# DCDmllm/AnyEdit

Hardware: AMD Instinct MI355X
Metric: edited-images/sec @512x512, 50 DDIM steps (higher is better)
Workload: dtype bf16; 1 GPU; configs[1]: AnySD (SD-1.5 UNet in=8 + task embedding/expert adapters) 512x512 bf16, 50 DDIM steps, batch=4/GPU, 3-branch CFG (UNet batch 12); images_per_gpu=4, ddim_steps=50, cfg_branches=3, hip_graph=True, parallelism=dp1 (image-sharded, no data-path collective)

## Files before the change

anyedit_amd/_lib.py:

```python
import ctypes
import os

import torch

_HERE = os.path.dirname(os.path.abspath(__file__))
LIB_PATH = os.environ.get("AE_LIB_PATH") or os.path.join(_HERE, "libanyedit_hip.so")

c_void_p, c_int, c_long, c_float = ctypes.c_void_p, ctypes.c_int, ctypes.c_long, ctypes.c_float

SIGNATURES = {
    "ae_version": [],
    "ae_last_error": [],
    "ae_device_arch": [ctypes.c_char_p, c_int],
    "ae_device_info": [ctypes.POINTER(c_int), ctypes.POINTER(c_long), ctypes.POINTER(c_int)],
    "ae_gemm_bf16": [c_void_p, c_long, c_void_p, c_long, c_int, c_void_p, c_long, c_void_p, c_long, c_int, c_int, c_int,
                     c_void_p, c_void_p, c_long, c_void_p, c_long, c_int, c_int, c_int, c_void_p, c_void_p],
    "ae_conv3x3_workspace_floats": [c_int, c_int, c_int, c_int, c_int, c_int, c_int],
    "ae_conv3x3_partials_bf16": [c_void_p, c_void_p, c_int, c_int, c_int, c_int, c_int, c_void_p, c_int, c_void_p, c_void_p],
    "ae_groupnorm_splitk_supported": [c_int, c_int, c_int, c_int, c_int],
    "ae_groupnorm_splitk_nhwc_bf16": [c_void_p, c_int, c_void_p, c_void_p, c_long, c_void_p, c_void_p, c_void_p, c_int, c_int, c_int, c_int, c_float, c_int, c_void_p],
    "ae_conv3x3_bf16": [c_void_p, c_void_p, c_void_p, c_void_p, c_long, c_void_p, c_void_p, c_int, c_int, c_int, c_int, c_int,
                        c_int, c_int, c_int, c_void_p, c_void_p, c_int, c_void_p],
    "ae_conv3x3_up2_bf16": [c_void_p, c_void_p, c_void_p, c_void_p, c_int, c_int, c_int, c_int, c_int, c_void_p, c_void_p],
    "ae_groupnorm_rows_per_chunk": [c_int, c_int],
# ... 16 lines not shown
    "ae_add_bf16": [c_void_p, c_void_p, c_void_p, c_long, c_void_p],
    "ae_axpy_bf16": [c_void_p, c_void_p, c_float, c_void_p, c_long, c_void_p],
    "ae_geglu_fwd_bf16": [c_void_p, c_void_p, c_long, c_int, c_void_p],
    "ae_geglu_bwd_bf16": [c_void_p, c_void_p, c_void_p, c_long, c_int, c_void_p],
    "ae_sumpool2x2_bf16": [c_void_p, c_void_p, c_int, c_int, c_int, c_int, c_void_p],
    "ae_colsum_bf16_f32": [c_void_p, c_void_p, c_int, c_int, c_long, c_void_p],
    "ae_mse_grad_f32": [c_void_p, c_void_p, c_void_p, c_long, c_float, c_void_p],
    "ae_adamw_f32": [c_void_p, c_void_p, c_void_p, c_void_p, c_long, c_float, c_float, c_float, c_float, c_float, c_int, c_float,
                     c_void_p],
    "ae_rowsum_f32": [c_void_p, c_void_p, c_int, c_long, c_void_p],
    "ae_scatter_add_rows_f32": [c_void_p, c_void_p, c_void_p, c_int, c_int, c_int, c_void_p],
    "ae_attn_fp8_workspace_bytes": [c_int, c_int, c_int, c_int, c_int],
    "ae_attn_fwd_fp8": [c_void_p, c_void_p, c_void_p, c_void_p, c_int, c_int, c_int, c_int, c_int] + [c_long] * 12 +
                       [c_float, c_void_p, c_void_p, c_int, c_int, c_void_p, c_long, c_void_p],
    "ae_ln_gemm_supported": [c_int, c_int, c_int, c_int],
    "ae_ln_gemm_bf16": [c_void_p, c_long, c_void_p, c_long, c_void_p, c_long, c_int, c_int, c_int, c_void_p, c_void_p, c_long, c_void_p, c_void_p,
                        c_float, c_int, c_void_p, c_void_p],
    "ae_gemm_ln_plan": [c_int, c_int, c_int, c_int, c_int],
    "ae_xattn_fused_supported": [c_int, c_int, c_int, c_int, c_int, c_int, c_int],
    "ae_xattn_fused_covers": [c_int, c_int, c_int, c_int, c_int, c_int, c_int],
    "ae_xattn_fused_kv_bytes": [],
    "ae_xattn_fused_bf16": [c_void_p, c_long, c_void_p, c_void_p, c_float, c_void_p, c_void_p, c_void_p, c_void_p, c_void_p, c_void_p, c_long, c_int, c_int, c_int, c_int,
                            c_float, c_void_p],
    "ae_ff_fused_supported": [c_int, c_int, c_int],
    "ae_ff_fused_bf16": [c_void_p, c_long, c_void_p, c_void_p, c_float, c_void_p, c_long, c_void_p, c_void_p, c_void_p, c_void_p, c_long,
                         c_void_p, c_long, c_void_p, c_void_p, c_long, c_void_p, c_void_p, c_long, c_int, c_int, c_int, c_void_p],
    "ae_gemm_ln_bf16": [c_void_p, c_long, c_void_p, c_long, c_void_p, c_long, c_int, c_int, c_int, c_void_p, c_void_p, c_long, c_int, c_void_p,
                        c_void_p, c_int, c_void_p, c_float, c_void_p],
    "ae_task_gate_bwd": [c_void_p, c_void_p, c_void_p, c_void_p, c_int, c_int, c_int, c_void_p, c_void_p],
    "ae_task_gate_wgrad": [c_void_p, c_void_p, c_void_p, c_void_p, c_void_p, c_int, c_int, c_int, c_int, c_void_p, c_void_p, c_void_p],
    "ae_expert_kv_fwd": [c_void_p, c_void_p, c_void_p, c_void_p, c_int, c_int, c_int, c_int, c_int, c_void_p],
    "ae_expert_kv_dgrad_slices": [c_int],
    "ae_expert_kv_dgrad": [c_void_p, c_void_p, c_void_p, c_void_p, c_int, c_int, c_int, c_int, c_int, c_void_p, c_void_p],
    "ae_expert_kv_wgrad": [c_void_p, c_void_p, c_void_p, c_void_p, c_int, c_int, c_int, c_int, c_int, c_void_p],
    "ae_transpose_last2": [c_void_p, c_void_p, c_int, c_int, c_int, c_int, c_int, c_int, c_void_p],
    "ae_concat_channels_bf16": [c_void_p, c_int, c_void_p, c_int, c_void_p, c_long, c_void_p],
    "ae_im2col3x3_c8_bf16": [c_void_p, c_void_p, c_int, c_int, c_int, c_void_p],
    "ae_split_channels_bf16": [c_void_p, c_int, c_int, c_void_p, c_void_p, c_long, c_int, c_int, c_void_p],
    "ae_timestep_embedding": [c_void_p, c_void_p, c_void_p, c_void_p, c_int, c_int, c_float, c_void_p],
    "ae_ddim_step_f32": [c_void_p, c_void_p, c_void_p, c_void_p, c_void_p, c_void_p, c_long, c_int, c_float, c_float, c_float,
                         c_float, c_float, c_float, c_float, c_float, c_void_p],
    "ae_ddim_encode_step_f32": [c_void_p, c_void_p, c_void_p, c_long, c_int, c_float, c_float, c_float, c_void_p],
    "ae_plms_combine_f32": [c_void_p, c_void_p, c_void_p, c_void_p, c_void_p, c_long, c_int, c_void_p],
    "ae_mask_blend_f32": [c_void_p, c_void_p, c_void_p, c_void_p, c_void_p, c_int, c_int, c_int, c_float, c_float, c_int, c_void_p],
    "ae_q_sample_f32": [c_void_p, c_void_p, c_void_p, c_void_p, c_void_p, c_int, c_long, c_void_p],
    "ae_silu_to_bf16": [c_void_p, c_int, c_void_p, c_long, c_void_p],
# ... 12 lines not shown
    "ae_ms_deform_attn_bwd_f32": [c_void_p] * 9 + [c_int] * 7 + [c_void_p],
    "ae_linear_f32": [c_void_p, c_long, c_void_p, c_long, c_void_p, c_void_p, c_long, c_int, c_int, c_int, c_void_p],
    "ae_dpm_multistep_f32": [c_void_p] * 5 + [c_long, c_int, c_float, c_int, c_int, c_float, c_float, c_int, c_float, c_float, c_float,
                             c_float, c_void_p],
    "ae_layernorm_act_bf16": [c_void_p, c_void_p, c_void_p, c_void_p, c_long, c_int, c_float, c_int, c_void_p],
    "ae_sam_pe_encode_f32": [c_void_p, c_void_p, c_void_p, c_void_p, c_void_p, c_int, c_int, c_float, c_float, c_float, c_void_p],
    "ae_sam_mask_downscale_bf16": [c_void_p] * 10 + [c_int, c_int, c_int, c_float, c_void_p],
    "ae_sam_mask_product_f32": [c_void_p, c_void_p, c_void_p, c_int, c_int, c_int, c_int, c_int, c_void_p],
    "ae_sam_postprocess_masks": [c_void_p, c_void_p, c_void_p] + [c_int] * 8 + [c_float, c_int, c_void_p],
    "ae_nms_sorted_f32": [c_void_p, c_void_p, c_int, c_float, c_void_p],
    "ae_sam_preprocess_f32": [c_void_p, c_int, c_void_p, c_int, c_int, c_int, c_int, c_int, c_void_p, c_void_p, c_void_p],
    "ae_patchify_f32_bf16": [c_void_p, c_void_p, c_int, c_int, c_int, c_int, c_int, c_void_p],
    "ae_mse_f32": [c_void_p, c_void_p, c_void_p, c_long, c_void_p],
    "ae_lincomb4_f32": [c_void_p, c_void_p, c_float, c_void_p, c_float, c_void_p, c_float, c_void_p, c_float, c_long, c_void_p],
    "ae_dpm_adaptive_err_f32": [c_void_p, c_void_p, c_void_p, c_float, c_float, c_int, c_long, c_void_p, c_void_p],
    "ae_task_gate": [c_void_p, c_void_p, c_void_p, c_void_p, c_int, c_int, c_int, c_int, c_void_p, c_void_p, c_void_p, c_void_p],
    "ae_attn_causal_short_bf16": [c_void_p, c_void_p, c_void_p, c_void_p, c_int, c_int, c_int, c_int] + [c_long] * 12 + [c_float, c_void_p],
    "ae_clip_embed_bf16": [c_void_p, c_int, c_void_p, c_void_p, c_void_p, c_int, c_int, c_int, c_int, c_int, c_void_p],
    "ae_bias_act_f32_bf16": [c_void_p, c_long, c_void_p, c_void_p, c_long, c_long, c_int, c_int, c_void_p],
    "ae_clip_pool_eos_bf16": [c_void_p, c_int, c_void_p, c_void_p, c_int, c_int, c_int, c_long, c_void_p],
}
_RESTYPES = {"ae_last_error": ctypes.c_char_p, "ae_groupnorm_workspace_floats": c_long, "ae_conv3x3_workspace_floats": c_long,
             "ae_groupnorm_bwd_workspace_floats": c_long, "ae_attn_fp8_workspace_bytes": c_long, "ae_attn_bwd_workspace_floats": c_long,
             "ae_xattn_fused_kv_bytes": c_long}


class AnyEditHipError(RuntimeError):
    pass


def _load():
    if not os.path.exists(LIB_PATH):
        raise ImportError(
            f"{LIB_PATH} is missing: the HIP extension is REQUIRED (no CPU/eager fallback exists). "
            "Build it with `python -c 'import __graft_entry__ as g; g.build()'` or `python anyedit_amd/build.py`.")
    lib = ctypes.CDLL(LIB_PATH)
    for name, argtypes in SIGNATURES.items():
        fn = getattr(lib, name)
        fn.argtypes = argtypes
        fn.restype = _RESTYPES.get(name, c_int)
    return lib


lib = _load()


def check(rc, what=""):
# ... 10 lines not shown
```

anyedit_amd/anysd/model.py:

```python
import torch
import torch.nn as nn

from anyedit_amd import ops
from anyedit_amd.cldm.model import trusted_torch_load
from anyedit_amd.ldm.modules.attention import BasicTransformerBlock

BF16 = torch.bfloat16

EDIT_TYPES = ["add", "remove", "replace", "color_alter", "appearance_alter", "material_alter", "action_change",
              "textual_change", "background_change", "tone_transfer", "style_change", "movement", "outpaint", "rotation_change",
              "resize", "implicit_change", "relation_change", "counting", "visual_reference", "visual_bbox", "visual_depth",
              "visual_scribble", "visual_segment", "visual_sketch", "visual_material_transfer"]


class ImageProjModel(nn.Module):

    def __init__(self, clip_dim=1280, cross_dim=768, tokens=4):
        super().__init__()
        self.tokens, self.cross_dim = tokens, cross_dim
        self.proj = nn.Linear(clip_dim, tokens * cross_dim)
        self.norm = nn.LayerNorm(cross_dim)

    def rows(self, ref_embeds):
        B = ref_embeds.shape[0]
# ... 34 lines not shown
    @torch.no_grad()
    def prepare_conditioning(self, encoder_hidden_states, ref_embeds, edit_code, ip_scale=None):
        B, L, Dc = encoder_hidden_states.shape
        dev = encoder_hidden_states.device
        te = self.task_embs.detach()[edit_code.long()]
        ctx = torch.cat([encoder_hidden_states.float(), te[:, None, :].float()], dim=1)
        context_rows = ctx.reshape(B * (L + 1), Dc).to(BF16).contiguous()
        probs, top1, top1p = self.route(edit_code)
        gate = top1p if ip_scale is None else top1p * ip_scale
        ip_rows = self.image_proj_model.rows(ref_embeds)
        T_ip = self.image_proj_model.tokens
        kv_cache = {}
        for blk, W in zip(self._blocks, self.adapter_modules):
            attn = blk.attn2
            kv_cache[id(attn)] = attn.project_kv(context_rows)
            Wm = W.detach()
            if Wm.dtype != torch.float32 or not Wm.is_contiguous():
                Wm = Wm.float().contiguous()
            kv_ip = ops.expert_kv(ip_rows, Wm, top1, T_ip)
            kv_cache[("adapter", id(attn))] = (kv_ip, gate.float().contiguous())
            img = attn.fused_kv_images(kv_cache[id(attn)], kv_cache[("adapter", id(attn))], B)
            if img is not None:
                kv_cache[("xattn_img", id(attn))] = img
        return context_rows, kv_cache

    @torch.no_grad()
    def denoise(self, x, timesteps, context_rows, kv_cache, emb_pack=None):
        return self.unet.forward_rows(x, timesteps, context_rows, kv_cache=kv_cache, emb_pack=emb_pack)

    def forward(self, noisy_latents, timesteps, encoder_hidden_states, image_embeds, edit_code):
        context_rows, kv_cache = self.prepare_conditioning(encoder_hidden_states, image_embeds, edit_code)
        return self.denoise(noisy_latents, timesteps, context_rows, kv_cache)
```

anyedit_amd/build.py:

```python
import hashlib
import os
import shutil
import subprocess
import sys

HERE = os.path.dirname(os.path.abspath(__file__))
CSRC = os.path.join(HERE, "csrc")
LIB = os.path.join(HERE, "libanyedit_hip.so")
SOURCES = ["c_api.hip", "gemm_conv.hip", "gemm_rowpanel.hip", "ff_fused.hip", "xattn_fused.hip", "attention.hip", "attention_fast.hip", "attention_fp8.hip", "attention_bwd.hip", "norm.hip", "elementwise.hip", "backward.hip", "gate.hip", "expert_kv.hip", "msda.hip",
           "sam_decoder.hip", "clip_text.hip"]
EXTRA = {"gemm_conv.hip": ["-fno-slp-vectorize"], "gemm_rowpanel.hip": ["-fno-slp-vectorize"], "ff_fused.hip": ["-fno-slp-vectorize"], "xattn_fused.hip": ["-fno-slp-vectorize"], "attention.hip": ["-ffinite-math-only"],
         "attention_fast.hip": ["-ffinite-math-only", "-fno-slp-vectorize"], "attention_fp8.hip": ["-ffinite-math-only"],
         "attention_bwd.hip": ["-ffinite-math-only"], "clip_text.hip": ["-ffinite-math-only"]}
FLAGS = ["--offload-arch=gfx950", "-O3", "-std=c++17", "-fPIC", "-fno-gpu-rdc", "-Wno-unused-result"]


def _hipcc():
    for c in (shutil.which("hipcc"), "/opt/rocm/bin/hipcc"):
        if c and os.path.exists(c):
            return c
    raise RuntimeError("hipcc not found: the HIP extension cannot be built")


def _digest():
    h = hashlib.sha256()
    for name in sorted(os.listdir(CSRC)):
        with open(os.path.join(CSRC, name), "rb") as f:
            h.update(name.encode() + f.read())
    h.update((" ".join(FLAGS) + repr(sorted(EXTRA.items()))).encode())
    return h.hexdigest()


def build_library(force=False, verbose=True, variant=None, extra_flags=None):
    lib = LIB if variant is None else os.path.join(HERE, f"libanyedit_hip_{variant}.so")
    extra = {k: list(v) for k, v in EXTRA.items()}
    for k, v in (extra_flags or {}).items():
# ... 46 lines not shown
```

anyedit_amd/ldm/modules/attention.py:

```python
import os

import torch
import torch.nn as nn

from anyedit_amd import ops
from anyedit_amd.ldm.util import default, exists
from anyedit_amd.ldm.modules.diffusionmodules.util import Linear, Conv2d, LayerNorm, checkpoint

BF16 = torch.bfloat16
_XATTN_FUSED = os.environ.get("AE_XATTN_FUSED", "0") != "0"
_FF_TAIL = os.environ.get("AE_FF_TAIL", "1") != "0"
_SEG2_160 = os.environ.get("AE_ATTN_SEG2_160", "1") != "0"


def zero_module(module):
    for p in module.parameters():
        p.detach().zero_()
    return module


class _GN6(nn.GroupNorm):

    def _affine(self):
        if ops.cache_stale(self, "_pk", self.weight, self.bias):
            self._pk = (self.weight.detach().float().contiguous(), self.bias.detach().float().contiguous())
        return self._pk

    def repack(self):
        self._pk = None

    def rows(self, x, B, HW, colstats=None):
        g, b = self._affine()
        return ops.groupnorm(x, g, b, B, HW, self.eps, silu=False, groups=self.num_groups, colstats=colstats)
# ... 120 lines not shown
        if ops.cache_stale(self, "_pk", self.to_q.weight, self.to_k.weight, self.to_v.weight):
            wq, wk, wv = (ops.pack_linear(m.weight) for m in (self.to_q, self.to_k, self.to_v))
            pk = {"dev": self.to_q.weight.device, "q": wq, "kv": torch.cat([wk, wv], 0).contiguous()}
            if wq.shape[1] == wk.shape[1]:
                pk["qkv"] = torch.cat([wq, wk, wv], 0).contiguous()
            self._pk = pk
        return self._pk

    def _packed_x(self):
        if ops.cache_stale(self, "_pkx", self.to_q.weight, self.to_out[0].weight, self.to_out[0].bias):
            bo = self.to_out[0].bias
            self._pkx = (ops.pack_xattn_wq(self.to_q.weight), ops.pack_xattn_wo(self.to_out[0].weight), None if bo is None else bo.detach().float().contiguous())
        return self._pkx

    def fused_kv_images(self, kv, adapter, B):
        if not _XATTN_FUSED or self.is_self or self.heads != 8 or self.dim_head != 40 or self.to_q.weight.shape[1] != 320:
            return None
        Nk = kv.shape[0] // B
        T = 0 if adapter is None else adapter[0].shape[0] // B
        if not (64 < Nk <= 80 and T <= 16):
            return None
        return ops.pack_xattn_kv(kv, None if adapter is None else adapter[0], B, Nk, T)

    def project_kv(self, ctx_rows):
        return ops.gemm(ctx_rows, self._packed()["kv"])

    def rows(self, x, B, N, context_rows=None, Nk=None, kv=None, key_mask=None, residual=None, adapter=None, norm=None, rowstats=None,
             out_rowstats=None, kv_img=None):
        h, d = self.heads, self.dim_head
        inner = h * d
        if kv_img is not None and kv is not None and norm is not None and residual is x and key_mask is None and out_rowstats is None:
            Nk_ = kv.shape[0] // B
            T_ = 0 if adapter is None else adapter[0].shape[0] // B
            if ops.xattn_fused_ok(x.shape[0], x.shape[1], h, d, N, Nk_, T_):
                wq_img, wo_img, bo = self._packed_x()
                g_, be_ = norm._affine()
                return ops.xattn_fused(x, g_, be_, norm.eps, wq_img, kv_img, None if adapter is None else adapter[1], wo_img, bo, N, Nk_, T_, self.scale)
        pk = self._packed()

        def proj(wname):
            if norm is None:
                return ops.gemm(x, pk[wname])
            if rowstats is not None and ops.ln_fold_plan(x.shape[0], pk[wname].shape[0], x.shape[1], ops.EPI_NONE, 2):
                wq, s, c = self._packed_ln(wname, norm)
                return ops.gemm_ln(x, rowstats, wq, s, c, norm.eps)
            g, be = norm._affine()
            return ops.ln_gemm(x, g, be, norm.eps, pk[wname])

        if context_rows is None and kv is None:
            qkv = proj("qkv")
            s = (N * 3 * inner, d, 3 * inner)
            o = ops.attention(qkv, qkv[:, inner:], qkv[:, 2 * inner:], B, h, N, N, d, self.scale, s, s, s, key_mask=key_mask)
        else:
            q = proj("q")
            if kv is None:
                kv = self.project_kv(context_rows)
            Nk = kv.shape[0] // B
            qs = (N * inner, d, inner)
            ks = (Nk * 2 * inner, d, 2 * inner)
            if adapter is not None and (d <= 96 or (d == 160 and _SEG2_160)) and key_mask is None:
                kv_ip, gate = adapter
                T_ip = kv_ip.shape[0] // B
                ks_ip = (T_ip * 2 * inner, d, 2 * inner)
                seg2 = (kv_ip, kv_ip[:, inner:], T_ip, ks_ip, ks_ip, gate)
                o = ops.attention(q, kv, kv[:, inner:], B, h, N, Nk, d, self.scale, qs, ks, ks, seg2=seg2)
            else:
                o = ops.attention(q, kv, kv[:, inner:], B, h, N, Nk, d, self.scale, qs, ks, ks, key_mask=key_mask)
                if adapter is not None:
                    kv_ip, gate = adapter
                    T_ip = kv_ip.shape[0] // B
                    ks_ip = (T_ip * 2 * inner, d, 2 * inner)
                    ops.attention(q, kv_ip, kv_ip[:, inner:], B, h, N, T_ip, d, self.scale, qs, ks_ip, ks_ip, out=o,
                                  out_scale=gate, accumulate=True)
        return self.to_out[0].rows(o.reshape(B * N, inner), residual=residual, rowstats=out_rowstats)

    def forward(self, x, context=None, mask=None):
        B, N, C = x.shape
        xr = x.reshape(B * N, C).to(BF16).contiguous()
        ctx = None
        if context is not None:
            ctx = context.reshape(-1, context.shape[-1]).to(BF16).contiguous()
        km = None
        if exists(mask):
# ... 59 lines not shown
        M, C = x.shape
        f1, f2, f3 = self._fold_plan(M, C)
        kv2, adapter, kv_img = None, None, None
        if kv_cache is not None and context_rows is not None and not (ops._TAPE is not None and ops._TAPE.active):
            kv_img = kv_cache.get(("xattn_img", id(self.attn2)))
        use_x = kv_img is not None and not f3 and ops.xattn_fused_ok(M, C, self.attn2.heads, self.attn2.dim_head, N, 78, 0)
        st2 = ops.rowstats_buffer(M, C, x.device) if (f2 and not use_x) else None
        st3 = ops.rowstats_buffer(M, C, x.device) if f3 else None
        x = self.attn1.rows(x, B, N, context_rows=c1, residual=x, norm=self.norm1, rowstats=rowstats if f1 else None, out_rowstats=st2)
        if kv_cache is not None and context_rows is not None:
            key = id(self.attn2)
            kv2 = kv_cache.get(key)
            if kv2 is None:
                kv2 = self.attn2.project_kv(context_rows)
                if not (ops._TAPE is not None and ops._TAPE.active):
                    kv_cache[key] = kv2
            adapter = kv_cache.get(("adapter", key))
            if callable(adapter):
                adapter = adapter()
            if kv_img is None and not f3 and not (ops._TAPE is not None and ops._TAPE.active):
                img = self.attn2.fused_kv_images(kv2, adapter, B)
                if img is not None:
                    kv_cache[("xattn_img", key)] = img
        x = self.attn2.rows(x, B, N, context_rows=context_rows, kv=kv2, residual=x, adapter=adapter, norm=self.norm2, rowstats=st2, out_rowstats=st3,
                            kv_img=kv_img if use_x else None)
        x = self.ff.rows(x, residual=x, norm=self.norm3, rowstats=st3, tail=tail)
        return x

    def forward(self, x, context=None):
        B, N, C = x.shape
        ctx = None if context is None else context.reshape(-1, context.shape[-1]).to(BF16).contiguous()
        y = self.rows(x.reshape(B * N, C).to(BF16).contiguous(), B, N, context_rows=ctx)
        return y.reshape(B, N, C).to(x.dtype)

    _forward = forward


class SpatialTransformer(nn.Module):

    def __init__(self, in_channels, n_heads, d_head, depth=1, dropout=0., context_dim=None, disable_self_attn=False,
                 use_linear=False, use_checkpoint=True):
        super().__init__()
        if exists(context_dim) and not isinstance(context_dim, list):
            context_dim = [context_dim] * depth
        if context_dim is None:
            context_dim = [None] * depth
        self.in_channels = in_channels
        inner_dim = n_heads * d_head
# ... 46 lines not shown
```

anyedit_amd/ops.py:

```python
import torch

import ctypes
import os
import threading

from ._lib import lib, check as _check

BF16 = torch.bfloat16
EPI_NONE, EPI_GELU, EPI_GEGLU, EPI_SILU, EPI_RELU = 0, 1, 2, 3, 4


def _s():
    return torch.cuda.current_stream().cuda_stream


def _p(t):
    return None if t is None else t.data_ptr()


_live = threading.local()


def _tmp(t):
    if t is not None:
# ... 281 lines not shown
    _chk(wo_img, BF16, "xattn_fused.wo_img", 3)
    _chk(kv_img, BF16, "xattn_fused.kv_img", 3)
    _chk(gamma, torch.float32, "xattn_fused.gamma", 1)
    _chk(beta, torch.float32, "xattn_fused.beta", 1)
    M, C = x.shape
    B = M // rows_per_sample
    if tuple(wq_img.shape) != (8, 48, 320) or tuple(wo_img.shape) != (4, 320, 112) or tuple(kv_img.shape) != (B, 8, 14848) or not (wq_img.is_contiguous() and wo_img.is_contiguous()
                                                                                                                                    and kv_img.is_contiguous()) or x.stride(1) != 1:
        raise ValueError(f"xattn_fused: x {tuple(x.shape)}, images {tuple(wq_img.shape)} / {tuple(wo_img.shape)} / {tuple(kv_img.shape)} do not fit together")
    if gate is not None:
        _chk(gate, torch.float32, "xattn_fused.gate", 1)
        if gate.numel() != B:
            raise ValueError("xattn_fused: one gate per sample")
    if bo is not None:
        _chk(bo, torch.float32, "xattn_fused.bo", 1)
    if out is None:
        out = torch.empty(M, C, dtype=BF16, device=x.device)
    _chk(out, BF16, "xattn_fused.out", 2)
    check(lib.ae_xattn_fused_bf16(_p(x), x.stride(0), _p(gamma), _p(beta), float(eps), _p(wq_img), _p(kv_img), _p(gate), _p(wo_img), _p(bo), _p(out), out.stride(0), M,
                                  rows_per_sample, Nk, T, float(scale), _s()), "ae_xattn_fused_bf16")
    return out


def colstats_buffer(M, N, device):
    return torch.empty((M + 31) // 32, N, 2, dtype=torch.float32, device=device)


_GN_COLSTATS = os.environ.get("AE_GN_COLSTATS", "1") != "0"


def want_colstats(HW):
    return _GN_COLSTATS and HW > 256 and HW % 32 == 0 and not (_TAPE is not None and _TAPE.active)


def gemm(a, w, bias=None, residual=None, addvec=None, rows_per_batch=0, epilogue=EPI_NONE, out_f32=False, a2=None, out=None, colstats=None,
         rowstats=None):
    if rowstats is not None:
        if _TAPE is not None and _TAPE.active:
            raise ValueError("gemm: row statistics are not recorded on the training tape (ln_fold_plan is False while it records)")
        if addvec is not None or a2 is not None or out_f32 or colstats is not None or epilogue != EPI_NONE:
            raise ValueError("gemm: rowstats goes with a plain bf16 GEMM (+bias, +residual) only")
        return _gemm_ln(a, w, bias, residual, EPI_NONE, out, rowstats, None, None, 0.0)
    if _TAPE is not None and _TAPE.active:
        return _TAPE.gemm(a, w, bias=bias, residual=residual, addvec=addvec, rows_per_batch=rows_per_batch, epilogue=epilogue, out_f32=out_f32, a2=a2, out=out)
    _chk(a, BF16, "gemm.a", 2)
    _chk(w, BF16, "gemm.w", 2)
# ... 1216 lines not shown
    return f"gemm_rowpanel_kernel<K=320,LN{',geglu' if epilogue == EPI_GEGLU else ''}>|M={M} N={N}", 2.0 * M * N * K, nb


def _gemm_ln_label(_r, a, w, bias, residual, epilogue, out, M, N, K, rowstats_out, ln_stats, nparts, ln_colsum, eps):
    nb = 2 * (M * K + N * K) + _r.numel() * 2 + (2 * M * N if residual is not None else 0)
    tag = "rowstats" if rowstats_out is not None else "LNfold"
    if _ROWPANEL and os.environ.get("AE_RP_FOLD", "1") != "0" and lib.ae_ln_gemm_supported(M, N, K, epilogue) and (rowstats_out is None or epilogue == EPI_NONE):
        return f"gemm_rowpanel_kernel<K=320,{tag}{',geglu' if epilogue == EPI_GEGLU else ''}>|M={M} N={N}", 2.0 * M * N * K, nb
    return f"gemm_kernel<{_tile_label(M, N, False, K, epilogue == EPI_GEGLU, True, xe2=rowstats_out is None)},dense,{tag}>|M={M} N={N} K={K}", 2.0 * M * N * K, float(nb)


def _up2_label(_r, x, w4, bias, B, H, W, **_):
    y = _r[0]
    M, Cout, Cin = x.shape[0], w4.shape[1], x.shape[1]
    t192 = (M // 192) * (Cout // 320) * 4 if (M % 192 == 0 and Cout % 320 == 0) else 0
    tl = "192x320" if t192 and t192 / (-(-t192 // 256) * 256) >= 0.85 else "128x128"
    nb = 2 * (x.numel() + 16 * Cin * Cout) + 2 * y.numel()
    return f"gemm_kernel<{tl},conv3x3,up2x2>|M={y.shape[0]} Cin={Cin} Cout={Cout}", 2.0 * y.shape[0] * Cout * 4 * Cin, float(nb)


conv3x3_up2 = _wrap_profiled(conv3x3_up2, _up2_label)
xattn_fused = _wrap_profiled(xattn_fused, lambda _r, x, gamma, beta, eps, wq_img, kv_img, gate, wo_img, bo, rows_per_sample, Nk, T, scale, out=None: (
    f"xattn_fused_kernel<C=320>|M={x.shape[0]} Nk={Nk}+{T}", 2.0 * x.shape[0] * 320 * (2 * 320 + 2 * (Nk + T)), float(2 * (3 * x.numel() + wq_img.numel() + wo_img.numel() + kv_img.numel()))))
ff_fused = _wrap_profiled(ff_fused, lambda _r, x, gamma, beta, eps, w1, b1, w2img, b2, residual=None, out=None, w3=None, b3=None, residual3=None, colstats=None: (
    f"ff_fused_kernel<C=320{',proj_out' if w3 is not None else ''}>|M={x.shape[0]} H={w1.shape[0] // 2}",
    2.0 * x.shape[0] * x.shape[1] * (3 * (w1.shape[0] // 2) + (x.shape[1] if w3 is not None else 0)),
    float(2 * (x.numel() * (2 + (residual is not None and residual is not x) + (residual3 is not None)) + w1.numel() + w2img.numel() + (w3.numel() if w3 is not None else 0))),
    2 if colstats is not None else 1))
_ln_gemm_fused = _wrap_profiled(_ln_gemm_launch, _ln_gemm_label)
_gemm_ln_launch = _wrap_profiled(_gemm_ln_launch, _gemm_ln_label)
gemm = _wrap_profiled(gemm, _gemm_label)
attention_fp8 = _wrap_profiled(attention_fp8, _attn8_label)
conv3x3 = _wrap_profiled(conv3x3, _conv_label)
conv3x3_partials = _wrap_profiled(conv3x3_partials, lambda _r, x, w, B, H, W, k_order=0: (
    f"gemm_kernel<{_tile_label(x.shape[0], w.shape[0], True, 9 * (-(-x.shape[1] // 64) * 64), False, x.shape[1] % 64 == 0)},conv3x3>|M={x.shape[0]} Cin={x.shape[1]} Cout={w.shape[0]} s1 partials",
    2.0 * x.shape[0] * w.shape[0] * 9 * x.shape[1], float(2 * (x.numel() + 9 * x.shape[1] * w.shape[0]) + 2 * x.shape[0] * w.shape[0]), 1))
groupnorm_splitk = _wrap_profiled(groupnorm_splitk, lambda _r, partials, *a, **k: (
    f"groupnorm(splitK fold)|rows={_r.shape[0]} C={_r.shape[1]}", 0.0, 2.0 * _r.numel() * 2, 1))
attention = _wrap_profiled(attention, _attn_label)
groupnorm = _wrap_profiled(groupnorm, _gn_label)
layernorm = _wrap_profiled(layernorm, _ln_label)
expert_kv = _wrap_profiled(expert_kv, lambda _r, x, W, experts, tokens: (
    f"expert_kv_fwd_kernel|rows={x.shape[0]} N={W.shape[1]} Dc={W.shape[2]}", 2.0 * x.shape[0] * W.shape[1] * W.shape[2], 4.0 * (x.shape[0] // tokens) * W.shape[1] * W.shape[2]))
expert_kv_dgrad = _wrap_profiled(expert_kv_dgrad, lambda _r, dy, W, experts, tokens: (
    f"expert_kv_dgrad_kernel|rows={dy.shape[0]} N={W.shape[1]} Dc={W.shape[2]}", 2.0 * dy.shape[0] * W.shape[1] * W.shape[2], 4.0 * (dy.shape[0] // tokens) * W.shape[1] * W.shape[2]))
expert_kv_wgrad = _wrap_profiled(expert_kv_wgrad, lambda _r, dy, x, experts, tokens, n_experts, out=None: (
# ... 2 lines not shown
```

include/anyedit_hip.h:

```cpp
#ifndef ANYEDIT_HIP_H
#define ANYEDIT_HIP_H

#ifdef __cplusplus
extern "C" {
#endif

#define AE_OK 0
#define AE_ERR_ARG (-1)
#define AE_ERR_LAUNCH (-2)
#define AE_ERR_UNSUPPORTED (-3)

#define AE_EPI_NONE 0
#define AE_EPI_GELU 1
#define AE_EPI_GEGLU 2
#define AE_EPI_SILU 3
#define AE_EPI_RELU 4

int ae_version(void);
const char* ae_last_error(void);
int ae_device_arch(char* buf, int n);
int ae_device_info(int* cus, long* hbm_bytes, int* clock_khz);

int ae_gemm_bf16(const void* A, long lda, const void* A2, long lda2, int Ksplit, const void* W, long ldw, void* C, long ldc,
                 int M, int N, int K, const float* bias, const void* residual, long ldr, const float* addvec, long addvec_ld,
                 int rows_per_batch, int epilogue, int out_f32, float* colstats, void* stream);

int ae_ln_gemm_supported(int M, int N, int K, int epilogue);
int ae_ln_gemm_bf16(const void* A, long lda, const void* W, long ldw, void* C, long ldc, int M, int N, int K, const float* bias,
                    const void* residual, long ldr, const float* ln_gamma, const float* ln_beta, float ln_eps, int epilogue,
                    float* colstats , void* stream);

int ae_gemm_ln_plan(int M, int N, int K, int epilogue, int mode);
int ae_gemm_ln_bf16(const void* A, long lda, const void* W, long ldw, void* C, long ldc, int M, int N, int K, const float* bias,
                    const void* residual, long ldr, int epilogue, float* rowstats_out, const float* ln_stats, int ln_parts,
                    const float* ln_colsum, float ln_eps, void* stream);

int ae_ff_fused_supported(int M, int C, int H);
int ae_ff_fused_bf16(const void* X, long ldx, const float* ln_gamma, const float* ln_beta, float ln_eps, const void* W1, long ldw1, const float* b1,
                     const void* W2img, const float* b2, const void* residual, long ldr, const void* W3, long ldw3, const float* b3,
                     const void* residual3, long ldr3, float* colstats, void* Y, long ldy, int M, int C, int H, void* stream);

int ae_xattn_fused_supported(int M, int C, int heads, int head_dim, int rows_per_sample, int Nk, int T);
int ae_xattn_fused_covers(int M, int C, int heads, int head_dim, int rows_per_sample, int Nk, int T);
long ae_xattn_fused_kv_bytes(void);
int ae_xattn_fused_bf16(const void* X, long ldx, const float* ln_gamma, const float* ln_beta, float ln_eps, const void* Wq_img, const void* KV_img, const float* gate,
                        const void* Wo_img, const float* bo, void* Y, long ldy, int M, int rows_per_sample, int Nk, int T, float scale, void* stream);

long ae_conv3x3_workspace_floats(int B, int H, int W, int Cin, int Cout, int stride, int upsample2x);
int ae_conv3x3_partials_bf16(const void* x, const void* w, int B, int H, int W, int Cin, int Cout, float* workspace, int k_order, int* splitk_out, void* stream);
int ae_conv3x3_bf16(const void* x, const void* w, const float* bias, const float* addvec, long addvec_ld, const void* residual,
                    void* y, int B, int H, int W, int Cin, int Cout, int stride, int upsample2x, int out_f32, float* workspace,
                    float* colstats , int k_order, void* stream);

int ae_conv3x3_up2_bf16(const void* x, const void* w4, const float* bias, void* y, int B, int H, int W, int Cin, int Cout,
                        float* colstats, void* stream);

int ae_groupnorm_rows_per_chunk(int HW, int C);
long ae_groupnorm_workspace_floats(int B, int HW, int C, int groups);
int ae_groupnorm_splitk_supported(int B, int HW, int C, int groups, int splitk);
int ae_groupnorm_splitk_nhwc_bf16(const float* partial, int splitk, const float* bias, const float* addvec, long addvec_ld, const float* gamma, const float* beta,
                                  void* y, int B, int HW, int C, int groups, float eps, int act, void* stream);
 * colstats / colstats2: optional per-channel slab statistics of x / x2 as written by the kernels that PRODUCED them (the `colstats`
 * output of ae_gemm_bf16 / ae_ln_gemm_bf16 / ae_conv3x3_bf16: [B*HW/32][C1][2] and [B*HW/32][C-C1][2]; HW % 32 == 0).  With them the
 * statistics pass over the activation is skipped: one block per (sample, group) folds the slab sums, then the apply launch runs.    */
int ae_groupnorm_nhwc_bf16(const void* x, const void* x2, int C1, const float* gamma, const float* beta, void* y, int B, int HW,
                           int C, int groups, float eps, int act, float* workspace, int* counters, float* stat_out,
                           const float* colstats, const float* colstats2, void* stream);

int ae_layernorm_bf16(const void* x, const float* gamma, const float* beta, void* y, int M, int C, float eps, void* stream);
// ... 126 lines not shown
```

Before: 6.437 edited-images/sec.

## Add short-context cross-attention kernel with packed K/V image and fused expert segment

Adds a HIP kernel for cross-attention with a short key set (text tokens plus up to 16 expert/adapter tokens). K/V are pre-packed once per sampling run into a per-head LDS-ready image, and the whole key set sits in shared memory. The text softmax and the gated expert softmax are computed together in one MFMA pass, which replaces the previous two-segment attention path. This removes repeated K/V loads and separate launches per segment, at the cost of a precomputed image per layer and bf16 rounding of the softmax probabilities.

```diff
diff --git a/anyedit_amd/_lib.py b/anyedit_amd/_lib.py
--- a/anyedit_amd/_lib.py
+++ b/anyedit_amd/_lib.py
@@ -62,6 +62,10 @@
     "ae_xattn_fused_kv_bytes": [],
     "ae_xattn_fused_bf16": [c_void_p, c_long, c_void_p, c_void_p, c_float, c_void_p, c_void_p, c_void_p, c_void_p, c_void_p, c_void_p, c_long, c_int, c_int, c_int, c_int,
                             c_float, c_void_p],
+    "ae_xattn_short_supported": [c_int, c_int, c_int],
+    "ae_xattn_short_image_elems": [c_int],
+    "ae_xattn_short_expert_slot": [c_int, c_int],
+    "ae_xattn_short_bf16": [c_void_p, c_long, c_void_p, c_long, c_void_p, c_void_p, c_int, c_int, c_int, c_int, c_int, c_int, c_float, c_void_p],
     "ae_ff_fused_supported": [c_int, c_int, c_int],
     "ae_ff_fused_bf16": [c_void_p, c_long, c_void_p, c_void_p, c_float, c_void_p, c_long, c_void_p, c_void_p, c_void_p, c_void_p, c_long,
                          c_void_p, c_long, c_void_p, c_void_p, c_long, c_void_p, c_void_p, c_long, c_int, c_int, c_int, c_void_p],
@@ -120,7 +124,7 @@
 }
 _RESTYPES = {"ae_last_error": ctypes.c_char_p, "ae_groupnorm_workspace_floats": c_long, "ae_conv3x3_workspace_floats": c_long,
              "ae_groupnorm_bwd_workspace_floats": c_long, "ae_attn_fp8_workspace_bytes": c_long, "ae_attn_bwd_workspace_floats": c_long,
-             "ae_xattn_fused_kv_bytes": c_long}
+             "ae_xattn_fused_kv_bytes": c_long, "ae_xattn_short_image_elems": c_long}
 
 
 class AnyEditHipError(RuntimeError):
diff --git a/anyedit_amd/anysd/model.py b/anyedit_amd/anysd/model.py
--- a/anyedit_amd/anysd/model.py
+++ b/anyedit_amd/anysd/model.py
@@ -80,6 +80,9 @@
             img = attn.fused_kv_images(kv_cache[id(attn)], kv_cache[("adapter", id(attn))], B)
             if img is not None:
                 kv_cache[("xattn_img", id(attn))] = img
+            img = attn.short_kv_image(kv_cache[id(attn)], kv_cache[("adapter", id(attn))], B)
+            if img is not None:
+                kv_cache[("xattn_short", id(attn))] = img
         return context_rows, kv_cache
 
     @torch.no_grad()
diff --git a/anyedit_amd/build.py b/anyedit_amd/build.py
--- a/anyedit_amd/build.py
+++ b/anyedit_amd/build.py
@@ -8,10 +8,11 @@
 CSRC = os.path.join(HERE, "csrc")
 LIB = os.path.join(HERE, "libanyedit_hip.so")
 SOURCES = ["c_api.hip", "gemm_conv.hip", "gemm_rowpanel.hip", "ff_fused.hip", "xattn_fused.hip", "attention.hip", "attention_fast.hip", "attention_fp8.hip", "attention_bwd.hip", "norm.hip", "elementwise.hip", "backward.hip", "gate.hip", "expert_kv.hip", "msda.hip",
-           "sam_decoder.hip", "clip_text.hip"]
+           "sam_decoder.hip", "clip_text.hip", "xattn_short.hip"]
 EXTRA = {"gemm_conv.hip": ["-fno-slp-vectorize"], "gemm_rowpanel.hip": ["-fno-slp-vectorize"], "ff_fused.hip": ["-fno-slp-vectorize"], "xattn_fused.hip": ["-fno-slp-vectorize"], "attention.hip": ["-ffinite-math-only"],
          "attention_fast.hip": ["-ffinite-math-only", "-fno-slp-vectorize"], "attention_fp8.hip": ["-ffinite-math-only"],
-         "attention_bwd.hip": ["-ffinite-math-only"], "clip_text.hip": ["-ffinite-math-only"]}
+         "attention_bwd.hip": ["-ffinite-math-only"], "clip_text.hip": ["-ffinite-math-only"],
+         "xattn_short.hip": ["-ffinite-math-only", "-fno-slp-vectorize"]}
 FLAGS = ["--offload-arch=gfx950", "-O3", "-std=c++17", "-fPIC", "-fno-gpu-rdc", "-Wno-unused-result"]
 
 
diff --git a/anyedit_amd/csrc/xattn_short.hip b/anyedit_amd/csrc/xattn_short.hip
--- /dev/null
+++ b/anyedit_amd/csrc/xattn_short.hip
@@ -0,0 +1,293 @@
+#include "common.hpp"
+
+
+namespace {
+
+constexpr int XS_SLOTS = 96;
+constexpr int XS_VROW = 104;
+constexpr int XS_CUS = 256;
+constexpr float XS_OUT = -1e30f;
+
+template <int D>
+struct XsGeom {
+    static constexpr int KS = (D + 31) / 32;
+    static constexpr int DT = (D + 15) / 16;
+    static constexpr int KROW = 32 * KS + 8;
+    static constexpr int KELEMS = XS_SLOTS * KROW;
+    static constexpr int IMG = KELEMS + 16 * DT * XS_VROW;
+};
+
+struct XsArgs {
+    const bf16_t* q;
+    const bf16_t* img;
+    const float* gate;
+    bf16_t* out;
+    long ldq;
+    int H, Nq, Nk, T, E0, NS;
+    float qscale;
+};
+
+__device__ __forceinline__ u32x4 lds16(const bf16_t* p) { return *reinterpret_cast<const u32x4*>(p); }
+
+__device__ __forceinline__ float xs_sum2(uint32_t w, float acc) {
+    union { uint32_t u; bf16x2_t b; } x, one;
+    x.u = w;
+    one.u = 0x3f803f80u;
+    return __builtin_amdgcn_fdot2_f32_bf16(x.b, one.b, acc, false);
+}
+
+template <int D, int KS>
+__device__ __forceinline__ void xs_load_q(u32x4 (&qf)[KS], const bf16_t* qb, long ldq, int Nq, int tile, int hh, int l15, int lg) {
+    int row = tile * 16 + l15;
+    row = row < Nq ? row : Nq - 1;
+    const bf16_t* p = qb + (long)row * ldq + hh * D;
+#pragma unroll
+    for (int ks = 0; ks < KS; ++ks) {
+        const int c = 4 * ks + lg;
+        qf[ks] = (u32x4){0u, 0u, 0u, 0u};
+        if (8 * (4 * ks + 3) < D || 8 * c < D) qf[ks] = *reinterpret_cast<const u32x4*>(p + 8 * c);
+    }
+}
+
+template <int D, int HG, int NW, bool UNET>
+__global__ __launch_bounds__(NW * 64) void xattn_short_kernel(const XsArgs a) {
+    using G = XsGeom<D>;
+    constexpr int KS = G::KS, DT = G::DT, KROW = G::KROW, IMG = G::IMG;
+    __shared__ __attribute__((aligned(16))) bf16_t smem[HG * IMG];
+    __shared__ __attribute__((aligned(16))) float sB1[XS_SLOTS], sB2[XS_SLOTS], sW2[XS_SLOTS];
+
+    const int tid = threadIdx.x, lane = tid & 63, wave = tid >> 6, l15 = lane & 15, lg = lane >> 4;
+    const int b = blockIdx.z, h0 = blockIdx.y * HG;
+    const int nh = (a.H - h0) < HG ? (a.H - h0) : HG;
+    const int ntiles = (a.Nq + 15) >> 4;
+    const int t0 = (int)((long)blockIdx.x * ntiles / gridDim.x), t1 = (int)((long)(blockIdx.x + 1) * ntiles / gridDim.x);
+    const int nitems = (t1 - t0) * nh;
+    const int HD = a.H * D;
+    const bf16_t* qb = a.q + (long)b * a.Nq * a.ldq + h0 * D;
+    bf16_t* ob = a.out + (long)b * a.Nq * HD + h0 * D;
+
+    const int step_t = NW / nh, step_h = NW % nh;
+    int item = wave, tile = t0 + wave / nh, hh = wave % nh;
+    int ntile = tile + step_t, nhh = hh + step_h;
+    if (nhh >= nh) { nhh -= nh; ++ntile; }
+    u32x4 qn[KS];
+    if (item < nitems) xs_load_q<D, KS>(qn, qb, a.ldq, a.Nq, tile, hh, l15, lg);
+
+    const int Nk = a.Nk, E0 = a.E0, E1 = a.E0 + a.T, NS = a.NS;
+    {
+        const u32x4* src = reinterpret_cast<const u32x4*>(a.img + ((long)b * a.H + h0) * IMG);
+        u32x4* dst = reinterpret_cast<u32x4*>(smem);
+        constexpr int U = (HG * (IMG / 8) + NW * 64 - 1) / (NW * 64);
+        u32x4 v[U];
+#pragma unroll
+        for (int u = 0; u < U; ++u)
+            if (tid + u * NW * 64 < nh * (IMG / 8)) v[u] = src[tid + u * NW * 64];
+#pragma unroll
+        for (int u = 0; u < U; ++u)
+            if (tid + u * NW * 64 < nh * (IMG / 8)) dst[tid + u * NW * 64] = v[u];
+        if (tid < XS_SLOTS) {
+            const bool text = tid < Nk, expert = tid >= E0 && tid < E1;
+            sB1[tid] = text ? 0.f : XS_OUT;
+            sB2[tid] = expert ? 0.f : XS_OUT;
+            sW2[tid] = expert ? 1.f : 0.f;
+        }
+    }
+    __syncthreads();
+
+    const float qscale = a.qscale;
+    const float gate = a.T > 0 ? a.gate[b] : 0.f;
+    int kind[6];
+#pragma unroll
+    for (int t = 0; t < 6; ++t) {
+        const bool has1 = 16 * t < Nk, has2 = a.T > 0 && 16 * t < E1 && 16 * t + 16 > E0;
+        kind[t] = UNET ? (t < 5 ? 1 : 2) : (has1 ? (has2 ? 3 : 1) : (has2 ? 2 : 0));
+    }
+    const bool has_expert = UNET || a.T > 0;
+
+    for (; item < nitems; item += NW) {
+        u32x4 qf[KS];
+#pragma unroll
+        for (int ks = 0; ks < KS; ++ks) qf[ks] = qn[ks];
+        if (item + NW < nitems) xs_load_q<D, KS>(qn, qb, a.ldq, a.Nq, ntile, nhh, l15, lg);
+
+        const bf16_t* sK = smem + hh * IMG;
+        const bf16_t* sV = sK + G::KELEMS;
+
+        f32x4 S[6];
+#pragma unroll
+        for (int t = 0; t < 6; ++t) {
+            S[t] = (f32x4){0.f, 0.f, 0.f, 0.f};
+            if (kind[t] != 0) {
+                if (kind[t] == 1 && !(UNET && t < 4)) S[t] = *reinterpret_cast<const f32x4*>(sB1 + 16 * t + 4 * lg);
+                if (kind[t] == 2) S[t] = *reinterpret_cast<const f32x4*>(sB2 + 16 * t + 4 * lg);
+#pragma unroll
+                for (int ks = 0; ks < KS; ++ks)
+                    S[t] = __builtin_amdgcn_mfma_f32_16x16x32_bf16(as_bf16x8(lds16(sK + (16 * t + l15) * KROW + 8 * (4 * ks + lg))), as_bf16x8(qf[ks]), S[t], 0, 0, 0);
+            }
+        }
+
+        float m1 = XS_OUT, m2 = XS_OUT;
+#pragma unroll
+        for (int t = 0; t < 6; ++t) {
+            if (kind[t] == 1) m1 = fmaxf(fmaxf(m1, fmaxf(S[t][0], S[t][1])), fmaxf(S[t][2], S[t][3]));
+            if (kind[t] == 2) m2 = fmaxf(fmaxf(m2, fmaxf(S[t][0], S[t][1])), fmaxf(S[t][2], S[t][3]));
+            if (kind[t] == 3) {
+                const f32x4 b1 = *reinterpret_cast<const f32x4*>(sB1 + 16 * t + 4 * lg), b2 = *reinterpret_cast<const f32x4*>(sB2 + 16 * t + 4 * lg);
+#pragma unroll
+                for (int r = 0; r < 4; ++r) {
+                    m1 = fmaxf(m1, S[t][r] + b1[r]);
+                    m2 = fmaxf(m2, S[t][r] + b2[r]);
+                }
+            }
+        }
+        m1 = fmaxf(m1, __shfl_xor(m1, 16, 64));
+        m1 = fmaxf(m1, __shfl_xor(m1, 32, 64));
+        if (has_expert) {
+            m2 = fmaxf(m2, __shfl_xor(m2, 16, 64));
+            m2 = fmaxf(m2, __shfl_xor(m2, 32, 64));
+        }
+        const float m1q = m1 * qscale, m2q = m2 * qscale;
+
+        float sum1 = 0.f, sum2 = 0.f;
+        uint32_t pw[6][2];
+#pragma unroll
+        for (int t = 0; t < 6; ++t) {
+            pw[t][0] = pw[t][1] = 0u;
+            if (kind[t] == 1) {
+                float e[4];
+#pragma unroll
+                for (int r = 0; r < 4; ++r) e[r] = __builtin_amdgcn_exp2f(__builtin_fmaf(S[t][r], qscale, -m1q));
+                pw[t][0] = pack_bf16x2(e[0], e[1]);
+                pw[t][1] = pack_bf16x2(e[2], e[3]);
+                sum1 = xs_sum2(pw[t][1], xs_sum2(pw[t][0], sum1));
+            }
+            if (kind[t] == 2) {
+#pragma unroll
+                for (int r = 0; r < 4; ++r) {
+                    S[t][r] = __builtin_amdgcn_exp2f(__builtin_fmaf(S[t][r], qscale, -m2q));
+                    sum2 += S[t][r];
+                }
+            }
+            if (kind[t] == 3) {
+                const f32x4 b1 = *reinterpret_cast<const f32x4*>(sB1 + 16 * t + 4 * lg), b2 = *reinterpret_cast<const f32x4*>(sB2 + 16 * t + 4 * lg);
+                float e1[4];
+#pragma unroll
+                for (int r = 0; r < 4; ++r) {
+                    e1[r] = __builtin_amdgcn_exp2f(__builtin_fmaf(S[t][r] + b1[r], qscale, -m1q));
+                    const float e2 = __builtin_amdgcn_exp2f(__builtin_fmaf(S[t][r] + b2[r], qscale, -m2q));
+                    sum2 += e2;
+                    S[t][r] = e1[r] + e2;
+                }
+                const uint32_t w0 = pack_bf16x2(e1[0], e1[1]), w1 = pack_bf16x2(e1[2], e1[3]);
+                sum1 = xs_sum2(w1, xs_sum2(w0, sum1));
+            }
+        }
+        sum1 += __shfl_xor(sum1, 16, 64);
+        sum1 += __shfl_xor(sum1, 32, 64);
+        const float inv1 = __builtin_amdgcn_rcpf(sum1);
+        if (has_expert) {
+            sum2 += __shfl_xor(sum2, 16, 64);
+            sum2 += __shfl_xor(sum2, 32, 64);
+            const float c2 = gate * sum1 * __builtin_amdgcn_rcpf(sum2);
+#pragma unroll
+            for (int t = 0; t < 6; ++t) {
+                if (kind[t] == 2) {
+                    pw[t][0] = pack_bf16x2(S[t][0] * c2, S[t][1] * c2);
+                    pw[t][1] = pack_bf16x2(S[t][2] * c2, S[t][3] * c2);
+                }
+                if (kind[t] == 3) {
+                    const f32x4 w2 = *reinterpret_cast<const f32x4*>(sW2 + 16 * t + 4 * lg);
+                    const float c2m1 = c2 - 1.f;
+                    pw[t][0] = pack_bf16x2(S[t][0] * __builtin_fmaf(w2[0], c2m1, 1.f), S[t][1] * __builtin_fmaf(w2[1], c2m1, 1.f));
+                    pw[t][1] = pack_bf16x2(S[t][2] * __builtin_fmaf(w2[2], c2m1, 1.f), S[t][3] * __builtin_fmaf(w2[3], c2m1, 1.f));
+                }
+            }
+        }
+        bf16x8_t pf[3];
+#pragma unroll
+        for (int s = 0; s < 3; ++s) pf[s] = as_bf16x8((u32x4){pw[2 * s][0], pw[2 * s][1], pw[2 * s + 1][0], pw[2 * s + 1][1]});
+
+        const bool rowok = tile * 16 + l15 < a.Nq;
+        bf16_t* op = ob + (long)(tile * 16 + l15) * HD + hh * D + 4 * DT * lg;
+        constexpr bool WIDE = (DT % 2 == 0) && ((4 * DT * 2) % 16 == 0) && (D % 16 == 0);
+        uint32_t held[2] = {0u, 0u};
+#pragma unroll
+        for (int dt = 0; dt < DT; ++dt) {
+            f32x4 acc = (f32x4){0.f, 0.f, 0.f, 0.f};
+#pragma unroll
+            for (int s = 0; s < 3; ++s)
+                if (UNET || 32 * s < NS)
+                    acc = __builtin_amdgcn_mfma_f32_16x16x32_bf16(as_bf16x8(lds16(sV + (16 * dt + l15) * XS_VROW + 32 * s + 8 * lg)), pf[s], acc, 0, 0, 0);
+            const uint32_t w0 = pack_bf16x2(acc[0] * inv1, acc[1] * inv1), w1 = pack_bf16x2(acc[2] * inv1, acc[3] * inv1);
+            if (WIDE) {
+                if (dt & 1) {
+                    if (rowok) *reinterpret_cast<u32x4*>(op + 4 * (dt - 1)) = (u32x4){held[0], held[1], w0, w1};
+                } else {
+                    held[0] = w0;
+                    held[1] = w1;
+                }
+            } else {
+                if (rowok && 4 * DT * lg + 4 * dt < D) *reinterpret_cast<u32x2*>(op + 4 * dt) = (u32x2){w0, w1};
+            }
+        }
+
+        tile = ntile;
+        hh = nhh;
+        ntile += step_t;
+        nhh += step_h;
+        if (nhh >= nh) { nhh -= nh; ++ntile; }
+    }
+}
+
+template <int D, int HG, int NW, int BPC>
+int xs_launch(const XsArgs& a, int B, hipStream_t stream) {
+    const bool unet = a.Nk > 64 && a.Nk <= 80 && a.T > 0 && a.E0 == 80;
+    const int ntiles = (a.Nq + 15) / 16;
+    const int hgroups = (a.H + HG - 1) / HG;
+    long nchunks = (long)XS_CUS * BPC / ((long)B * hgroups);
+    const long by_items = (long)ntiles * (a.H < HG ? a.H : HG) / NW;
+    if (nchunks > by_items) nchunks = by_items;
+    if (nchunks > ntiles) nchunks = ntiles;
+    if (nchunks < 1) nchunks = 1;
+    if (unet)
+        hipLaunchKernelGGL((xattn_short_kernel<D, HG, NW, true>), dim3((unsigned)nchunks, (unsigned)hgroups, (unsigned)B), dim3(NW * 64), 0, stream, a);
+    else
+        hipLaunchKernelGGL((xattn_short_kernel<D, HG, NW, false>), dim3((unsigned)nchunks, (unsigned)hgroups, (unsigned)B), dim3(NW * 64), 0, stream, a);
+    return ae_check_launch("ae_xattn_short_bf16");
+}
+
+}
+
+extern "C" int ae_xattn_short_supported(int D, int Nk, int T) {
+    return ((D == 40 || D == 80 || D == 160) && Nk >= 1 && T >= 0 && T <= 16 && Nk + T <= XS_SLOTS) ? 1 : 0;
+}
+
+extern "C" int ae_xattn_short_expert_slot(int Nk, int T) {
+    const int al = (Nk + 15) / 16 * 16;
+    return (T > 0 && (al + T + 31) / 32 == (Nk + T + 31) / 32) ? al : Nk;
+}
+
+extern "C" long ae_xattn_short_image_elems(int D) {
+    return D == 40 ? XsGeom<40>::IMG : D == 80 ? XsGeom<80>::IMG : D == 160 ? XsGeom<160>::IMG : 0;
+}
+
+extern "C" int ae_xattn_short_bf16(const void* q, long ldq, const void* kv_img, long img_stride, const float* gate, void* out, int B, int H, int Nq, int Nk, int T, int D,
+                                   float scale, void* stream) {
+    AE_REQUIRE(q && kv_img && out, "ae_xattn_short_bf16: null pointer");
+    AE_REQUIRE(ae_xattn_short_supported(D, Nk, T), "ae_xattn_short_bf16: unsupported shape D=%d Nk=%d T=%d (D in {40, 80, 160}, Nk >= 1, T <= 16, Nk + T <= 96)", D, Nk, T);
+    AE_REQUIRE(T == 0 || gate, "ae_xattn_short_bf16: an expert segment needs its gate");
+    AE_REQUIRE(B >= 1 && B <= 65535 && H >= 1 && H <= 65535 && Nq >= 1 && Nq <= (1 << 27), "ae_xattn_short_bf16: B=%d H=%d Nq=%d out of range", B, H, Nq);
+    AE_REQUIRE(ldq >= (long)H * D && ldq % 8 == 0, "ae_xattn_short_bf16: q row stride %ld (at least H*D = %ld, a multiple of 8 elements)", ldq, (long)H * D);
+    AE_REQUIRE(img_stride == ae_xattn_short_image_elems(D), "ae_xattn_short_bf16: image of %ld elements per head, head dim %d takes %ld", img_stride, D,
+               ae_xattn_short_image_elems(D));
+    AE_REQUIRE(((uintptr_t)q & 15) == 0 && ((uintptr_t)kv_img & 15) == 0 && ((uintptr_t)out & 15) == 0, "ae_xattn_short_bf16: 16-byte alignment");
+    AE_REQUIRE(out != q, "ae_xattn_short_bf16: in-place operation is not supported");
+    AE_REQUIRE(scale > 0.f && scale < 1e30f, "ae_xattn_short_bf16: scale");
+    XsArgs a{};
+    a.q = (const bf16_t*)q; a.img = (const bf16_t*)kv_img; a.gate = gate; a.out = (bf16_t*)out; a.ldq = ldq;
+    a.H = H; a.Nq = Nq; a.Nk = Nk; a.T = T; a.E0 = ae_xattn_short_expert_slot(Nk, T); a.NS = (a.E0 + T + 31) / 32 * 32; a.qscale = scale * 1.4426950408889634f;
+    hipStream_t st = (hipStream_t)stream;
+    if (D == 40) return xs_launch<40, 4, 16, 1>(a, B, st);
+    if (D == 80) return xs_launch<80, 2, 8, 2>(a, B, st);
+    return xs_launch<160, 1, 8, 2>(a, B, st);
+}
diff --git a/anyedit_amd/ldm/modules/attention.py b/anyedit_amd/ldm/modules/attention.py
--- a/anyedit_amd/ldm/modules/attention.py
+++ b/anyedit_amd/ldm/modules/attention.py
@@ -9,6 +9,7 @@
 
 BF16 = torch.bfloat16
 _XATTN_FUSED = os.environ.get("AE_XATTN_FUSED", "0") != "0"
+_XATTN_SHORT = os.environ.get("AE_XATTN_SHORT", "1") != "0"
 _FF_TAIL = os.environ.get("AE_FF_TAIL", "1") != "0"
 _SEG2_160 = os.environ.get("AE_ATTN_SEG2_160", "1") != "0"
 
@@ -175,11 +176,20 @@
             return None
         return ops.pack_xattn_kv(kv, None if adapter is None else adapter[0], B, Nk, T)
 
+    def short_kv_image(self, kv, adapter, B):
+        if not _XATTN_SHORT or self.is_self:
+            return None
+        Nk = kv.shape[0] // B
+        T = 0 if adapter is None else adapter[0].shape[0] // B
+        if not ops.xattn_short_ok(self.dim_head, Nk, T):
+            return None
+        return ops.pack_xattn_short_kv(kv, None if adapter is None else adapter[0], B, self.heads, self.dim_head, Nk, T)
+
     def project_kv(self, ctx_rows):
         return ops.gemm(ctx_rows, self._packed()["kv"])
 
     def rows(self, x, B, N, context_rows=None, Nk=None, kv=None, key_mask=None, residual=None, adapter=None, norm=None, rowstats=None,
-             out_rowstats=None, kv_img=None):
+             out_rowstats=None, kv_img=None, xs_img=None):
         h, d = self.heads, self.dim_head
         inner = h * d
         if kv_img is not None and kv is not None and norm is not None and residual is x and key_mask is None and out_rowstats is None:
@@ -211,7 +221,11 @@
             Nk = kv.shape[0] // B
             qs = (N * inner, d, inner)
             ks = (Nk * 2 * inner, d, 2 * inner)
-            if adapter is not None and (d <= 96 or (d == 160 and _SEG2_160)) and key_mask is None:
+            T_x = 0 if adapter is None else adapter[0].shape[0] // B
+            if xs_img is not None and _XATTN_SHORT and key_mask is None and not (ops._TAPE is not None and ops._TAPE.active) and ops.xattn_short_ok(d, Nk, T_x) \
+                    and tuple(xs_img.shape[:2]) == (B, h):
+                o = ops.xattn_short(q, xs_img, None if adapter is None else adapter[1], B, h, N, Nk, T_x, d, self.scale)
+            elif adapter is not None and (d <= 96 or (d == 160 and _SEG2_160)) and key_mask is None:
                 kv_ip, gate = adapter
                 T_ip = kv_ip.shape[0] // B
                 ks_ip = (T_ip * 2 * inner, d, 2 * inner)
@@ -317,8 +331,11 @@
                 img = self.attn2.fused_kv_images(kv2, adapter, B)
                 if img is not None:
                     kv_cache[("xattn_img", key)] = img
+        xs_img = None
+        if kv_cache is not None and context_rows is not None and kv2 is not None and not (ops._TAPE is not None and ops._TAPE.active):
+            xs_img = kv_cache.get(("xattn_short", id(self.attn2)))
         x = self.attn2.rows(x, B, N, context_rows=context_rows, kv=kv2, residual=x, adapter=adapter, norm=self.norm2, rowstats=st2, out_rowstats=st3,
-                            kv_img=kv_img if use_x else None)
+                            kv_img=kv_img if use_x else None, xs_img=xs_img)
         x = self.ff.rows(x, residual=x, norm=self.norm3, rowstats=st3, tail=tail)
         return x
 
diff --git a/anyedit_amd/ops.py b/anyedit_amd/ops.py
--- a/anyedit_amd/ops.py
+++ b/anyedit_amd/ops.py
@@ -327,6 +327,62 @@
     return out
 
 
+def xattn_short_ok(D, Nk, T):
+    return bool(lib.ae_xattn_short_supported(D, Nk, T))
+
+
+def pack_xattn_short_kv(kv, kv_ip, B, H, D, Nk, T, out=None):
+    _chk(kv, BF16, "pack_xattn_short_kv.kv", 2)
+    if not xattn_short_ok(D, Nk, T):
+        raise ValueError(f"pack_xattn_short_kv: D={D} Nk={Nk} T={T} is outside the kernel's envelope")
+    inner = H * D
+    if tuple(kv.shape) != (B * Nk, 2 * inner) or (T > 0 and (kv_ip is None or tuple(kv_ip.shape) != (B * T, 2 * inner))):
+        raise ValueError(f"pack_xattn_short_kv: kv {tuple(kv.shape)} / expert kv {None if kv_ip is None else tuple(kv_ip.shape)} do not fit B={B} H={H} D={D} Nk={Nk} T={T}")
+    dev = kv.device
+    KS, DT = -(-D // 32), -(-D // 16)
+    krow = 32 * KS + 8
+    rows = kv.reshape(B, Nk, 2, H, D)
+    slots = torch.zeros(B, 96, 2, H, D, dtype=BF16, device=dev)
+    slots[:, :Nk] = rows
+    if T > 0:
+        e0 = lib.ae_xattn_short_expert_slot(Nk, T)
+        slots[:, e0:e0 + T] = kv_ip.to(BF16).reshape(B, T, 2, H, D)
+    kimg = torch.zeros(B, H, 96, krow, dtype=BF16, device=dev)
+    kimg[..., :D] = slots[:, :, 0].permute(0, 2, 1, 3)
+    col = torch.arange(96, device=dev)
+    s_, g_, j_ = col >> 5, (col >> 3) & 3, col & 7
+    slot_of_col = 32 * s_ + 16 * (j_ >> 2) + 4 * g_ + (j_ & 3)
+    drow = torch.arange(16 * DT, device=dev)
+    d_of_row = 4 * DT * ((drow >> 2) & 3) + 4 * (drow >> 4) + (drow & 3)
+    vt = torch.cat([slots[:, :, 1].permute(0, 2, 3, 1), torch.zeros(B, H, 1, 96, dtype=BF16, device=dev)], 2)
+    vimg = torch.zeros(B, H, 16 * DT, 104, dtype=BF16, device=dev)
+    vimg[..., :96] = vt[:, :, torch.where(d_of_row < D, d_of_row, torch.full_like(d_of_row, D))][..., slot_of_col]
+    img = torch.cat([kimg.reshape(B, H, -1), vimg.reshape(B, H, -1)], 2)
+    assert img.shape[2] == lib.ae_xattn_short_image_elems(D)
+    if out is not None:
+        out.copy_(img)
+        return out
+    return img.contiguous()
+
+
+def xattn_short(q, kv_img, gate, B, H, Nq, Nk, T, D, scale, out=None):
+    _chk(q, BF16, "xattn_short.q", 2)
+    _chk(kv_img, BF16, "xattn_short.kv_img", 3)
+    if q.shape[0] != B * Nq or q.shape[1] < H * D or q.stride(1) != 1 or not kv_img.is_contiguous() or tuple(kv_img.shape[:2]) != (B, H):
+        raise ValueError(f"xattn_short: q {tuple(q.shape)} / images {tuple(kv_img.shape)} do not fit B={B} H={H} Nq={Nq} D={D}")
+    if gate is not None:
+        _chk(gate, torch.float32, "xattn_short.gate", 1)
+        if gate.numel() != B or not gate.is_contiguous():
+            raise ValueError("xattn_short: one gate per sample")
+    if out is None:
+        out = torch.empty(B, Nq, H * D, dtype=BF16, device=q.device)
+    _chk(out, BF16, "xattn_short.out", 3)
+    if tuple(out.shape) != (B, Nq, H * D) or not out.is_contiguous():
+        raise ValueError("xattn_short: out must be a contiguous [B, Nq, H*D] tensor")
+    check(lib.ae_xattn_short_bf16(_p(q), q.stride(0), _p(kv_img), kv_img.shape[2], _p(gate), _p(out), B, H, Nq, Nk, T, D, float(scale), _s()), "ae_xattn_short_bf16")
+    return out
+
+
 def colstats_buffer(M, N, device):
     return torch.empty((M + 31) // 32, N, 2, dtype=torch.float32, device=device)
 
@@ -1589,6 +1645,8 @@
 conv3x3_up2 = _wrap_profiled(conv3x3_up2, _up2_label)
 xattn_fused = _wrap_profiled(xattn_fused, lambda _r, x, gamma, beta, eps, wq_img, kv_img, gate, wo_img, bo, rows_per_sample, Nk, T, scale, out=None: (
     f"xattn_fused_kernel<C=320>|M={x.shape[0]} Nk={Nk}+{T}", 2.0 * x.shape[0] * 320 * (2 * 320 + 2 * (Nk + T)), float(2 * (3 * x.numel() + wq_img.numel() + wo_img.numel() + kv_img.numel()))))
+xattn_short = _wrap_profiled(xattn_short, lambda _r, q, kv_img, gate, B, H, Nq, Nk, T, D, scale, out=None: (
+    f"xattn_short_kernel<D={D}>|Nq={Nq} Nk={Nk}+{T}", 4.0 * B * H * Nq * (Nk + T) * D, 2.0 * B * H * D * (2 * Nq + 2 * (Nk + T))))
 ff_fused = _wrap_profiled(ff_fused, lambda _r, x, gamma, beta, eps, w1, b1, w2img, b2, residual=None, out=None, w3=None, b3=None, residual3=None, colstats=None: (
     f"ff_fused_kernel<C=320{',proj_out' if w3 is not None else ''}>|M={x.shape[0]} H={w1.shape[0] // 2}",
     2.0 * x.shape[0] * x.shape[1] * (3 * (w1.shape[0] // 2) + (x.shape[1] if w3 is not None else 0)),
diff --git a/include/anyedit_hip.h b/include/anyedit_hip.h
--- a/include/anyedit_hip.h
+++ b/include/anyedit_hip.h
@@ -45,6 +45,12 @@
 long ae_xattn_fused_kv_bytes(void);
 int ae_xattn_fused_bf16(const void* X, long ldx, const float* ln_gamma, const float* ln_beta, float ln_eps, const void* Wq_img, const void* KV_img, const float* gate,
                         const void* Wo_img, const float* bo, void* Y, long ldy, int M, int rows_per_sample, int Nk, int T, float scale, void* stream);
+
+int ae_xattn_short_supported(int D, int Nk, int T);
+long ae_xattn_short_image_elems(int D);
+int ae_xattn_short_expert_slot(int Nk, int T);
+int ae_xattn_short_bf16(const void* q, long ldq, const void* kv_img, long img_stride, const float* gate, void* out, int B, int H, int Nq, int Nk, int T, int D, float scale,
+                        void* stream);
 
 long ae_conv3x3_workspace_floats(int B, int H, int W, int Cin, int Cout, int stride, int upsample2x);
 int ae_conv3x3_partials_bf16(const void* x, const void* w, int B, int H, int W, int Cin, int Cout, float* workspace, int k_order, int* splitk_out, void* stream);
```

New measurement: 6.448 edited-images/sec (median of 6 runs). Within noise of the previous version (+0.2%).
